# awslabs/flowgger

Hardware: AMD Instinct MI355X
Metric: log lines/sec (RFC5424, 256B avg) at 1/2/4/8 MI355X; achieved HBM GB/s (higher is better)
Workload: dtype u8

## Files before the change

flowgger_amd/csrc/fg_pipeline.hpp:

```cpp
#pragma once
#include "fg_device.hpp"
#include "fg_plan_policy.hpp"
#include "fg_sparse_need.hpp"
#include "fg_wave.hpp"

namespace fg {

using u32x4 = unsigned int __attribute__((ext_vector_type(4)));

__device__ __forceinline__ uint32_t eq_flags(uint32_t x, uint32_t pat) {
    uint32_t s = ((x & 0x7F7F7F7Fu) ^ pat) + 0x7F7F7F7Fu;
    return ~(s | x) & 0x80808080u;
}
__device__ __forceinline__ uint32_t range_flags(uint32_t x) {
    uint32_t l = x & 0x7F7F7F7Fu;
    uint32_t ge33 = l + 0x5F5F5F5Fu;
    uint32_t le126 = l + 0x01010101u;
    return ge33 & ~le126 & ~x & 0x80808080u;
}
__device__ __forceinline__ uint32_t ctrl_flags(uint32_t x) {
    uint32_t ge32 = (x & 0x7F7F7F7Fu) + 0x60606060u;
    return ~(ge32 | x) & 0x80808080u;
}
__device__ __forceinline__ uint32_t gather16(uint32_t f0, uint32_t f1, uint32_t f2, uint32_t f3) {
// ... 210 lines not shown
    uint32_t* ticket = nullptr;
    uint32_t ticket_base = 0;
    uint32_t taper0 = kNoTaper, taper1 = kNoTaper, taper2 = kNoTaper;
};

#define FG_STREAM_AUX 2
__device__ __forceinline__ uint4 stream_load(const uint4* p) {
    typedef uint32_t nt4 __attribute__((ext_vector_type(4)));
    const nt4 v = __builtin_nontemporal_load(reinterpret_cast<const nt4*>(p));
    return make_uint4(v.x, v.y, v.z, v.w);
}

template <class F, class = void>
struct tail_batch { static constexpr int value = 4; };
template <class F>
struct tail_batch<F, decltype((void)F::kTailBatch)> { static constexpr int value = F::kTailBatch; };

template <class F, class = void>
struct defer_row_store { static constexpr bool value = true; };
template <class F>
struct defer_row_store<F, decltype((void)F::kDeferRowStore)> { static constexpr bool value = F::kDeferRowStore; };

constexpr uint32_t kHeadCap = 1024;
template <class F, class = void>
struct head_cap { static constexpr uint32_t value = kHeadCap; };
template <class F>
struct head_cap<F, decltype((void)F::kHeadBytes)> { static constexpr uint32_t value = F::kHeadBytes; };

constexpr uint32_t kSparseHandful = 4;

template <int NB, bool PROF, class F, bool HEAD = false, uint32_t SPARSE = 0>
__device__ __forceinline__ void persistent_loop(const uint8_t* __restrict__ bytes, const uint64_t* __restrict__ offsets,
                                                uint64_t n, const DevTables& t, uint32_t tile_cap, uint32_t L, uint64_t chunk_lines,
                                                unsigned long long* prof, uint64_t* stash_base, F& fmt, FrameArgs fr) {
    static_assert(!HEAD || F::kClasses <= 1, "HEAD staging classifies one stage-A byte class at most");
    static_assert(SPARSE == 0 || (!HEAD && F::kClasses == 0), "the sparse window builds its need bitmap where a stage-A class bitmap would lie");
    static_assert(SPARSE % 16u == 0 && SPARSE <= 112u, "a line's run of chunks (at most (H + 4 + 14) / 16 + 1) must fit two bitmap words at any shift");
    const uint64_t kChunkLines = chunk_lines;
    extern __shared__ __attribute__((aligned(16))) uint8_t smem[];
    uint16_t* bm16 = reinterpret_cast<uint16_t*>(smem + tile_cap + 64u);
    const uint32_t bm_stride = tile_cap / 16u + 16u;
    uint4* dst = reinterpret_cast<uint4*>(smem);
    const uint32_t lane = threadIdx.x;
    const uint64_t G = gridDim.x;
    uint64_t* stash = stash_base ? stash_base + (uint64_t)blockIdx.x * (kStashEntries * kStashWords * kWave) : nullptr;

    const bool dyn = fr.ticket != nullptr;
    uint32_t tk_raw = 0;
    bool tk_pending = false;
    auto draw_ticket = [&]() {
        if (lane == 0u) tk_raw = __hip_atomic_fetch_add(fr.ticket, 1u, __ATOMIC_RELAXED, __HIP_MEMORY_SCOPE_AGENT);
        tk_pending = true;
    };
    uint64_t chunk = blockIdx.x;
    uint64_t p, hi_line;
    chunk_range(chunk, kChunkLines, fr.taper0, fr.taper1, fr.taper2, n, &p, &hi_line);
    if (dyn && p < n) draw_ticket();

    auto load_offsets = [&](uint64_t q, uint64_t* o0, uint64_t* o1) {
        const uint64_t li = q + lane;
        const bool in = lane < L && li < hi_line;
        *o0 = offsets[in ? li : hi_line];
        *o1 = offsets[in ? li + 1 : hi_line];
    };
    auto geometry = [&](uint64_t q, uint64_t o0, uint64_t o1, uint32_t* nl, uint64_t* a0, uint32_t* span) {
        const uint64_t left = hi_line - q;
        const uint32_t avail = left < (uint64_t)L ? (uint32_t)left : L;
        const uint32_t lo_l = (uint32_t)__builtin_amdgcn_readfirstlane((int)(uint32_t)o0);
        const uint32_t lo_h = (uint32_t)__builtin_amdgcn_readfirstlane((int)(uint32_t)(o0 >> 32));
        const uint64_t lo = (uint64_t)lo_l | ((uint64_t)lo_h << 32);
        *a0 = lo & ~15ull;
        const unsigned long long fit = __ballot(lane < avail && (o1 - *a0) <= (uint64_t)tile_cap);
        uint32_t cnt = fit == ~0ull ? 64u : (uint32_t)__builtin_ctzll(~fit);
        if (cnt == 0u) cnt = 1u;
        *nl = cnt;
        const uint32_t last = cnt - 1u;
        const uint32_t hi_l = (uint32_t)__builtin_amdgcn_readlane((int)(uint32_t)o1, (int)last);
        const uint32_t hi_h = (uint32_t)__builtin_amdgcn_readlane((int)(uint32_t)(o1 >> 32), (int)last);
        const uint64_t hi = (uint64_t)hi_l | ((uint64_t)hi_h << 32);
        const uint64_t want = hi - *a0;
        *span = want > tile_cap ? tile_cap : (uint32_t)((want + 15ull) & ~15ull);
    };
    auto load_window = [&](uint64_t a0, uint32_t span, u32x4* v) {
        __amdgpu_buffer_rsrc_t rsrc =
            __builtin_amdgcn_make_buffer_rsrc(const_cast<uint8_t*>(bytes + a0), (short)0, (int)span, 0x00020000);
#pragma unroll
        for (int k = 0; k < NB; ++k) v[k] = __builtin_amdgcn_raw_buffer_load_b128(rsrc, (int)(lane * 16u + k * 1024u), 0, FG_STREAM_AUX);
    };
    const uint32_t sparse_tail = fr.strip != FG_FRAME_NONE ? kSparseTailFramed : kSparseTailPlain;
// ... 70 lines not shown
    if (lane < 2u) ent_state[lane] = 0u;
    if (p >= hi_line) return;
    uint64_t o0, o1, a0 = 0;
    uint32_t span, nl, st = 0, tb = 0, last2 = 0;
    load_offsets(p, &o0, &o1);
    u32x4 v[NB];
    if constexpr (HEAD) {
        geometry_head(p, o0, o1, &nl, &span, &st, &tb);
        load_window_head(o0, st, v);
        last2 = load_last2(o0, o1);
    } else if constexpr (SPARSE != 0) {
        geometry(p, o0, o1, &nl, &a0, &span);
        uint32_t vo[NB];
        sparse_offsets(a0, span, nl, o0, o1, false, vo);
        load_window_sparse(a0, span, vo, v);
    } else {
        geometry(p, o0, o1, &nl, &a0, &span);
        load_window(a0, span, v);
    }
    bool dense = false, dense_next = false, dense_then = false;
    RowOut pend{};
    uint64_t pend_li = 0;
    bool pend_valid = false;
    uint64_t acc0 = 0, acc1 = 0, acc2 = 0, acc3 = 0, iters = 0, tm0 = 0, tm1 = 0, tm2 = 0, tm3 = 0;
    const uint32_t ablate = PROF ? (uint32_t)prof[5] : 0u;
    const uint32_t term4 = fr.strip == FG_FRAME_LINE ? 0x0A0A0A0Au : fr.strip == FG_FRAME_NUL ? 0u : wv::kNoTerm;

    for (;;) {
        uint64_t pn = p + nl;
        if (pn >= hi_line) {
            if (dyn) {
                if (!tk_pending) draw_ticket();
                const uint32_t tk = (uint32_t)__builtin_amdgcn_readfirstlane((int)tk_raw);
                chunk = (uint64_t)(uint32_t)(tk - fr.ticket_base) + G;
                tk_pending = false;
                chunk_range(chunk, kChunkLines, fr.taper0, fr.taper1, fr.taper2, n, &pn, &hi_line);
                if (pn < n) draw_ticket();
            } else {
                chunk += G;
                chunk_range(chunk, kChunkLines, kNoTaper, kNoTaper, kNoTaper, n, &pn, &hi_line);
            }
        }
        const bool more = pn < n;
        uint64_t no0 = 0, no1 = 0;
        if (more) load_offsets(pn, &no0, &no1);
        if (PROF) {
            tm0 = __builtin_amdgcn_s_memtime();
            __builtin_amdgcn_s_waitcnt(0x0F70);
            tm1 = __builtin_amdgcn_s_memtime();
        }
        FG_MARK(A);
        const uint32_t nchunk = span >> 4;
        const uint32_t nrow = HEAD ? nl : (nchunk + kWave - 1u) / kWave;
        if constexpr (HEAD) {
#pragma unroll
            for (int k = 0; k < NB; ++k) {
                if ((uint32_t)k < nl) {
                    const uint32_t tk = (uint32_t)__builtin_amdgcn_readlane((int)tb, k), sk = (uint32_t)__builtin_amdgcn_readlane((int)st, k);
                    if (lane * 16u < sk) {
                        const uint4 q = make_uint4(v[k][0], v[k][1], v[k][2], v[k][3]);
                        dst[(tk >> 4) + lane] = q;
                        if constexpr (F::kClasses != 0) F::classify_store(q, bm16, (tk >> 4) + lane, bm_stride, term4);
                    }
                }
            }
            constexpr uint32_t HB = tail_batch<F>::value >= 8 ? 8u : 4u;
            for (uint32_t r0 = NB; r0 < nl; r0 += HB) {
                uint4 w[HB];
                uint32_t tk[HB], sk[HB];
#pragma unroll
                for (uint32_t j = 0; j < HB; ++j) {
                    const uint32_t r = r0 + j < nl ? r0 + j : nl - 1u;
                    const uint32_t lo = (uint32_t)__builtin_amdgcn_readlane((int)(uint32_t)o0, (int)r);
                    const uint32_t hi = (uint32_t)__builtin_amdgcn_readlane((int)(uint32_t)(o0 >> 32), (int)r);
                    tk[j] = (uint32_t)__builtin_amdgcn_readlane((int)tb, (int)r);
                    sk[j] = (uint32_t)__builtin_amdgcn_readlane((int)st, (int)r);
                    const uint64_t b = ((uint64_t)lo | ((uint64_t)hi << 32)) & ~15ull;
                    __amdgpu_buffer_rsrc_t rsrc = __builtin_amdgcn_make_buffer_rsrc(const_cast<uint8_t*>(bytes + b), (short)0, (int)sk[j], 0x00020000);
                    const u32x4 x = __builtin_amdgcn_raw_buffer_load_b128(rsrc, (int)(lane * 16u), 0, FG_STREAM_AUX);
                    w[j] = make_uint4(x[0], x[1], x[2], x[3]);
                }
#pragma unroll
                for (uint32_t j = 0; j < HB; ++j)
                    if (lane * 16u < sk[j]) {
                        dst[(tk[j] >> 4) + lane] = w[j];
                        if constexpr (F::kClasses != 0) F::classify_store(w[j], bm16, (tk[j] >> 4) + lane, bm_stride, term4);
                    }
            }
        } else {
#pragma unroll
        for (int k = 0; k < NB; ++k) {
            if ((uint32_t)k < nrow) {
                uint32_t idx = k * kWave + lane;
                uint4 q = make_uint4(v[k][0], v[k][1], v[k][2], v[k][3]);
                dst[idx] = q;
                F::classify_store(q, bm16, idx, bm_stride, idx < nchunk ? term4 : wv::kPastSpan);
            }
        }
        }
        if (!HEAD && nrow > (uint32_t)NB) {
            const uint4* __restrict__ src = reinterpret_cast<const uint4*>(bytes + a0);
            const uint32_t last = nchunk - 1u;
            constexpr int TB = tail_batch<F>::value;
            for (uint32_t c0 = NB * kWave; c0 < nchunk; c0 += kWave * TB) {
                uint4 w[TB];
#pragma unroll
                for (int k = 0; k < TB; ++k) {
                    const uint32_t idx = c0 + k * kWave + lane;
                    w[k] = stream_load(src + (idx < last ? idx : last));
                }
#pragma unroll
                for (int k = 0; k < TB; ++k) {
                    if (k == 0 || c0 + k * kWave < nchunk) {
                        const uint32_t idx = c0 + k * kWave + lane, ci = idx < last ? idx : last;
                        dst[ci] = w[k];
                        F::classify_store(w[k], bm16, ci, bm_stride, term4);
                    }
                }
            }
            if constexpr (SPARSE != 0) __builtin_amdgcn_s_waitcnt(0x0F70);
        }
        __builtin_amdgcn_sched_barrier(0);
        FG_MARK(S);
        if (PROF) {
            __builtin_amdgcn_s_waitcnt(0xC07F);
// ... 261 lines not shown
```

flowgger_amd/csrc/fg_plan_policy.hpp:

```cpp
#pragma once
#include <stdint.h>

#include "../../include/fg_hip.h"
#include "fg_sparse_need.hpp"

#if defined(__HIPCC__)
#define FG_POLICY_HD __host__ __device__
#else
#define FG_POLICY_HD
#endif

namespace fg {

constexpr uint32_t kNoTaper = 0xFFFFFFFFu;

FG_POLICY_HD inline void chunk_range(uint64_t c, uint64_t chunk, uint32_t t0, uint32_t t1, uint32_t t2, uint64_t n, uint64_t* lo,
                                     uint64_t* hi) {
    uint64_t base = 0, first = 0, sz = chunk;
    if (c >= t0) {
        base = (uint64_t)t0 * sz, first = t0, sz >>= 1;
        if (c >= t1) {
            base += (uint64_t)(t1 - t0) * sz, first = t1, sz >>= 1;
            if (c >= t2) base += (uint64_t)(t2 - t1) * sz, first = t2, sz >>= 1;
        }
// ... 54 lines not shown
        if (chunk < L) chunk = L;
    }
    if (chunk < 1u) chunk = 1u;
    p.chunk = chunk;
    p.chunks = (n + chunk - 1) / chunk;
    if (lo.flags & (FG_LO_TAPER_1 | FG_LO_TAPER_2)) taper = ((lo.flags & FG_LO_TAPER_1) ? 1u : 0u) + ((lo.flags & FG_LO_TAPER_2) ? 2u : 0u);
    if (taper > 3u) taper = 3u;
    if (tickets && taper && !(lo.flags & FG_LO_NO_TAPER)) {
        uint64_t m = n / (2u * chunk);
        if (m > blocks) m = blocks;
        uint32_t levels = 0;
        while (levels < taper && (chunk >> (levels + 1u)) >= g) ++levels;
        if (m >= 1u && levels >= 1u && p.chunks + 4u * m < 0xFFFFFFF0ull) {
            const uint64_t t0 = (n - m * chunk) / chunk;
            p.taper[0] = (uint32_t)t0;
            if (levels >= 2u) p.taper[1] = (uint32_t)(t0 + m);
            if (levels >= 3u) p.taper[2] = (uint32_t)(t0 + 2u * m);
            p.chunks = count_chunks(chunk, p.taper, n);
        }
    }
    p.blocks = (uint32_t)(blocks > p.chunks ? p.chunks : blocks);
    p.tickets = tickets;
    return p;
}

constexpr int kWindowKiB = 20;
constexpr uint32_t kMaxTile = 57344;

constexpr uint32_t tile_lds(uint32_t tile, uint32_t classes = 1) { return tile + 64u + (tile / 16u + 16u) * 2u * classes; }

constexpr uint32_t kShortLineTile = 17408;
static_assert(tile_lds(kShortLineTile) <= 160u * 1024u / 8u, "eight waves per CU");
static_assert(tile_lds(kShortLineTile + 1024u) > 160u * 1024u / 8u, "the largest such tile");

constexpr uint64_t kHeadFromLen = 768, kPairsFromLen = 320;
struct Variant { bool head, pairs; };
inline Variant pick_variant(uint64_t avg_len, uint32_t flags) {
    return Variant{(flags & FG_LO_FORCE_HEAD) || (avg_len >= kHeadFromLen && !(flags & FG_LO_NO_HEAD)),
                   (flags & FG_LO_SD_PAIRS) || (avg_len >= kPairsFromLen && !(flags & FG_LO_SD_WALK))};
}
#if !defined(FG_SPARSE_DEFAULT)
#define FG_SPARSE_DEFAULT 1
#endif
constexpr bool kSparseDefault = FG_SPARSE_DEFAULT != 0;
inline bool pick_sparse(uint64_t avg_len, uint32_t flags, const Variant& v) {
    if (v.head || v.pairs) return false;
    return (flags & FG_LO_FORCE_SPARSE) || (kSparseDefault && avg_len >= kSparseFromLen && !(flags & FG_LO_NO_SPARSE));
}
inline bool gelf_group_fits_3k(uint64_t avg_len) { return 8u * avg_len * 17u / 16u + 256u <= 3072u; }
inline bool gelf_const_3k(uint64_t avg_len, const fg_launch_opts& lo) {
    return gelf_group_fits_3k(avg_len) && !lo.tile_cap && !(lo.flags & FG_LO_GELF_GENERIC);
}

struct PlanFormat {
    uint32_t max_lines = 64;
    uint32_t n_classes = 1;
    uint32_t (*extra_for)(uint32_t tile, uint32_t lines) = nullptr;
    uint32_t (*extra_tile)(uint32_t tile) = nullptr;
    uint32_t default_tile = 0;
    uint32_t default_chunk = 0;
    uint32_t ticket_from = 2;
    uint32_t taper = 1;
    PlanFormat& lines(uint32_t v) { max_lines = v; return *this; }
    PlanFormat& classes(uint32_t v) { n_classes = v; return *this; }
    PlanFormat& lds_for(uint32_t (*f)(uint32_t, uint32_t)) { extra_for = f; return *this; }
    PlanFormat& lds_tile(uint32_t (*f)(uint32_t)) { extra_tile = f; return *this; }
// ... 73 lines not shown
```

flowgger_amd/csrc/fg_rfc5424.hip:

```cpp
#include <cstdio>
#include <cstdlib>

#include "fg_fused.hpp"
#include "fg_sd2.hpp"
#include "fg_tsfast.hpp"

namespace fg {

enum : uint32_t {
    E_OK = 0,
    E_BOM = 1,
    E_BRACKETS = 2,
    E_INVPRI = 3,
    E_NOVER = 4,
    E_BADVER = 5,
    E_NOTS = 6,
    E_BADTS = 7,
    E_NOHOST = 8,
    E_NOAPP = 9,
    E_NOPROC = 10,
    E_NOMSGID = 11,
    E_NODATA = 12,
    E_NOMSG = 13,
    E_MALFORMED = 14,
    E_NOSD = 15,
    E_SDFMT = 16,
    E_NOBRACKET = 17
};

struct Row {
    uint32_t status = E_OK;
    uint32_t facility = 0xFF, severity = 0xFF, flags = 0;
    double ts = 0.0;
    uint32_t off[6];
    uint32_t len[6];
    uint32_t data0 = 0;
    uint32_t n_ent = 0;
};


template <class R>
__device__ __forceinline__ uint32_t find_space(R& rd, uint32_t q, uint32_t len) {
    while (q < len && rd.byte(q) != ' ') ++q;
    return q;
}

template <bool EMIT, class R>
__device__ __forceinline__ uint32_t sd_walk(R& rd, uint32_t pos, uint32_t len, uint32_t* msg_at, uint32_t* n_ent,
                            const DevTables& t, uint32_t slot) {
    uint32_t cnt = 0;
    for (;;) {
        uint32_t s = pos + 1;
        uint32_t sp = find_space(rd, s, len);
        if (sp >= len) return E_NOSD;
        if (EMIT) {
            t.ent_name[slot + cnt] = fg_span{s, sp - s};
            t.ent_val[slot + cnt] = 0;
            t.ent_type[slot + cnt] = FG_T_SDID;
            t.ent_flags[slot + cnt] = 0;
        }
        ++cnt;
        uint32_t st = 0, name_s = 0, name_e = 0, val_s = 0, esc_seen = 0;
        uint32_t i = sp + 1;
        uint32_t after = 0;
        for (; i < len; ++i) {
            uint32_t c = rd.byte(i);
            if (st == 3) {
                if (c == '\\') {
                    st = 4;
                    esc_seen = 1;
                } else if (c == '"') {
                    if (EMIT) {
                        t.ent_name[slot + cnt] = fg_span{name_s, name_e - name_s};
                        t.ent_val[slot + cnt] = (uint64_t)val_s | ((uint64_t)(i - val_s) << 32);
                        t.ent_type[slot + cnt] = FG_T_STRING;
                        t.ent_flags[slot + cnt] = esc_seen ? FG_EF_VAL_ESC : 0;
                    }
                    ++cnt;
                    st = 0;
                }
            } else if (st == 4) {
                st = 3;
            } else {
                bool is_name = (c - 33u) <= 93u && c != '"' && c != '=' && c != ']';
                if (st == 0) {
                    if (c == ' ' || c == '"') {
                    } else if (c == ']') {
                        after = i + 1;
                        break;
                    } else if (is_name) {
                        st = 1;
                        name_s = i;
                    } else {
                        return E_SDFMT;
                    }
                } else if (st == 1) {
                    if (is_name) {
                    } else if (c == '=') {
                        name_e = i;
                        st = 2;
                    } else {
                        return E_SDFMT;
                    }
                } else {
                    if (c != '"') return E_SDFMT;
                    st = 3;
                    val_s = i + 1;
                    esc_seen = 0;
                }
// ... 142 lines not shown
struct Fast {
    uint32_t route;
    uint32_t no_ts;
    uint32_t ts_ok;
    uint32_t rest;
    uint32_t t0, te;
    uint32_t d0;
    uint32_t c7;
    uint32_t e, s;
    uint32_t start_ok;
};

__device__ __forceinline__ uint32_t fast_rfc3339(const Tile& T, uint32_t base, const uint32_t* hdr, uint32_t t0, uint32_t L,
                                                 double* out) {
    const uint32_t a = base + t0;
    const uint32_t s = t0 - 4u;
    uint32_t r[9];
#pragma unroll
    for (int k = 0; k < 9; ++k) r[k] = __builtin_amdgcn_alignbyte(hdr[k + 2], hdr[k + 1], s);
    return fast_rfc3339_core(r, L, [&](uint32_t pos, uint32_t* z0, uint32_t* z1) { load8(T, a + pos, z0, z1); }, out);
}

__device__ __forceinline__ uint32_t take_space(uint64_t& lo, uint64_t& hi, uint32_t none, uint32_t& found) {
    const bool in_lo = lo != 0, in_hi = hi != 0;
    const uint32_t p = in_lo ? (uint32_t)__builtin_ctzll(lo) : in_hi ? 64u + (uint32_t)__builtin_ctzll(hi) : none;
    const uint64_t lo2 = lo & (lo - 1ull), hi2 = hi & (hi - 1ull);
    hi = in_lo ? hi : hi2;
    lo = lo2;
    found += (in_lo || in_hi) ? 1u : 0u;
    return p;
}

constexpr uint32_t kNoLastByte = 0xFFFFFFFFu;
__device__ __forceinline__ Fast parse_line_fast(const Tile& T, uint32_t base, uint32_t len, Row& r, uint32_t last_byte, uint32_t vis) {
    Fast f;
    uint32_t l0 = last_byte, l1;
    if (last_byte == kNoLastByte) load8(T, base + (len ? len - 1u : 0u), &l0, &l1);
    uint32_t hdr[33];
    {
        const uint32_t d = base >> 2, sft = base & 3u;
        uint32_t raw[34];
#pragma unroll
        for (int k = 0; k < 34; ++k) raw[k] = T.w[d + k];
#pragma unroll
        for (int k = 0; k < 33; ++k) hdr[k] = __builtin_amdgcn_alignbyte(raw[k + 1], raw[k], sft);
    }
    const uint32_t h0 = hdr[0], h1 = hdr[1];

    const uint32_t c1 = ((h0 >> 8) & 0xFFu) - '0', c2 = ((h0 >> 16) & 0xFFu) - '0', c3 = (h0 >> 24) - '0';
    const bool d2 = c2 <= 9u, d3 = d2 && c3 <= 9u;
    const uint32_t nd = 1u + (d2 ? 1u : 0u) + (d3 ? 1u : 0u);
    uint32_t pri = c1;
    pri = d2 ? pri * 10u + c2 : pri;
    pri = d3 ? pri * 10u + c3 : pri;
    const uint64_t hh = (((uint64_t)h1 << 32) | h0) >> (8u * (1u + nd));
    const uint32_t sp0 = 3u + nd;
    const bool shape = (h0 & 0xFFu) == '<' && c1 <= 9u && pri <= 255u && (uint32_t)(hh & 0xFFFFu) == (('1' << 8) | '>') &&
                       sp0 <= len;
    f.no_ts = sp0 == len ? 1u : 0u;
    f.route = (!shape || (sp0 < len && (uint32_t)((hh >> 16) & 0xFFu) != ' ')) ? R_GENERIC : 0u;
    r.facility = pri >> 3;
    r.severity = pri & 7u;

    uint64_t lo, hi;
    {
        uint32_t m[8];
#pragma unroll
        for (int k = 0; k < 8; ++k)
            m[k] = gather16(eq_flags(hdr[4 * k], 0x20202020u), eq_flags(hdr[4 * k + 1], 0x20202020u),
                            eq_flags(hdr[4 * k + 2], 0x20202020u), eq_flags(hdr[4 * k + 3], 0x20202020u));
        lo = (uint64_t)(m[0] | (m[1] << 16)) | ((uint64_t)(m[2] | (m[3] << 16)) << 32);
        hi = (uint64_t)(m[4] | (m[5] << 16)) | ((uint64_t)(m[6] | (m[7] << 16)) << 32);
    }
    {
        const uint64_t lo_keep = vis < 64u ? (1ull << (vis & 63u)) - 1ull : ~0ull;
        const uint64_t hi_keep = vis < 64u ? 0ull : vis < 128u ? (1ull << ((vis - 64u) & 63u)) - 1ull : ~0ull;
        lo &= lo_keep & ~((2ull << sp0) - 1ull);
        hi &= hi_keep;
    }
    uint32_t found = 0;
    const uint32_t s1 = take_space(lo, hi, len, found);
    const uint32_t s2 = take_space(lo, hi, len, found);
    const uint32_t s3 = take_space(lo, hi, len, found);
    const uint32_t s4 = take_space(lo, hi, len, found);
    const uint32_t s5 = take_space(lo, hi, len, found);
    f.route |= (found < 5u && len > 128u) ? R_GENERIC : 0u;

    f.t0 = sp0 + 1u;
    f.te = s1;
    {
        const uint32_t ok = fast_rfc3339(T, base, hdr, f.t0, s1 - f.t0, &r.ts);
        f.ts_ok = ok == 1u ? 1u : 0u;
        f.route |= ok == 2u ? R_TS_SLOW : 0u;
    }
    r.off[S_HOST] = s1 + 1u;
    r.len[S_HOST] = s2 - s1 - 1u;
    r.off[S_APP] = s2 + 1u;
    r.len[S_APP] = s3 - s2 - 1u;
    r.off[S_PROC] = s3 + 1u;
    r.len[S_PROC] = s4 - s3 - 1u;
    r.off[S_MSGID] = s4 + 1u;
    r.len[S_MSGID] = s5 - s4 - 1u;
    const uint32_t d0 = s5 + 1u;
    f.d0 = d0;
    f.rest = found < 5u ? E_NOHOST + found : d0 >= len ? E_NOMSG : E_OK;

    uint32_t m0, m1;
    load8(T, base + (d0 < len ? d0 : 0u), &m0, &m1);
    const uint32_t c = m0 & 0xFFu;
    f.c7 = c;
    const bool live = !f.no_ts && f.rest == E_OK;
    f.route |= (live && c != '-') ? R_TAIL : 0u;
    const uint32_t last = l0 & 0xFFu;
    const bool end_plain = last > 0x20u && last < 0x80u;
    f.e = len;
    const uint32_t cA = (m0 >> 8) & 0xFFu, cB = (m0 >> 16) & 0xFFu;
    const uint32_t s = d0 + 1u;
    const bool one_sp = s + 1u < len && cA == ' ' && cB > 0x20u && cB < 0x80u;
    const bool no_sp = s < len && cA > 0x20u && cA < 0x80u;
// ... 50 lines not shown
    constexpr bool EMIT = MODE == SD_EMIT;
    LdsReader rd(T.w, base);
    uint32_t cnt = 0;
    uint32_t wpos = (base + 3u) & ~3u;
    bool rec_ok = true;
    auto record = [&](uint64_t rec, uint32_t consumed) {
        if (rec_ok) {
            if (wpos + 8u <= base + consumed) {
                tile_w[wpos >> 2] = (uint32_t)rec;
                tile_w[(wpos >> 2) + 1u] = (uint32_t)(rec >> 32);
                wpos += 8u;
            } else {
                rec_ok = false;
            }
        }
    };
    for (;;) {
        const uint32_t s = pos + 1;
        uint32_t sp = s;
        for (;;) {
            if (sp >= len) return E_NOSD;
            uint32_t w[4];
            load16(T, base + sp, w);
            const uint32_t avail = len - sp < 16u ? len - sp : 16u;
            const uint32_t hit = gather16(eq_flags(w[0], 0x20202020u), eq_flags(w[1], 0x20202020u), eq_flags(w[2], 0x20202020u),
                                          eq_flags(w[3], 0x20202020u)) & ((1u << avail) - 1u);
            if (hit) {
                sp += (uint32_t)__builtin_ctz(hit);
                break;
            }
            sp += avail;
        }
        if (EMIT) {
            t.ent_name[slot + cnt] = fg_span{s, sp - s};
            t.ent_val[slot + cnt] = 0;
            t.ent_type[slot + cnt] = FG_T_SDID;
            t.ent_flags[slot + cnt] = 0;
        }
        if (MODE == SD_STASH) record(stash_pack(s, sp - s, 0, 0, 1), sp + 1u);
        ++cnt;
        uint32_t status = E_OK;
        uint32_t i = sp + 1;
        bool in_value = false;
        uint32_t name_s = 0, name_e = 0, val_s = 0, cur = 0, esc_seen = 0;
        uint32_t close_at = 0;
        for (;;) {
            uint32_t w0 = i, start = 0;
            if (in_value) {
                const uint32_t p = find_bit(T.bm, base, cur, len);
                if (p >= len) {
                    status = E_NOBRACKET;
                    break;
                }
                w0 = p;
                start = 1;
            } else if (i >= len) {
                status = E_NOBRACKET;
                break;
            }
            uint32_t w[4];
            load16(T, base + w0, w);
            if (in_value) {
                if ((w[0] & 0xFFu) == '\\') {
                    esc_seen = 1;
                    cur = w0 + 2;
                    continue;
                }
                if (EMIT) {
                    t.ent_name[slot + cnt] = fg_span{name_s, name_e - name_s};
                    t.ent_val[slot + cnt] = (uint64_t)val_s | ((uint64_t)(w0 - val_s) << 32);
                    t.ent_type[slot + cnt] = FG_T_STRING;
                    t.ent_flags[slot + cnt] = esc_seen ? FG_EF_VAL_ESC : 0;
                }
                if (MODE == SD_STASH) record(stash_pack(name_s, name_e - name_s, w0 - val_s, esc_seen, 0), w0 + 1u);
                ++cnt;
                in_value = false;
            }
            const uint32_t avail = len - w0 < 16u ? len - w0 : 16u;
            const uint32_t inside = (1u << avail) - 1u;
            const WinMasks m = window_masks(w);
            const uint32_t from = ~((1u << start) - 1u);
            const uint32_t stop = ~m.skip & from & inside;
            if (stop == 0) {
                i = w0 + avail;
                continue;
            }
            const uint32_t i0 = (uint32_t)__builtin_ctz(stop);
            if ((m.rb >> i0) & 1u) {
                close_at = w0 + i0;
                break;
            }
            if (!((m.name >> i0) & 1u)) {
                status = E_SDFMT;
                break;
            }
            const uint32_t after_name = ~m.name & ~((1u << i0) - 1u) & 0xFFFFu;
            const uint32_t e0 = after_name ? (uint32_t)__builtin_ctz(after_name) : 16u;
            if (e0 + 1u < avail) {
                if (!((m.eq >> e0) & 1u) || !((m.quote >> (e0 + 1u)) & 1u)) {
                    status = E_SDFMT;
                    break;
                }
                name_s = w0 + i0;
                name_e = w0 + e0;
                val_s = name_e + 2u;
// ... 105 lines not shown
    const bool valid = c.valid;
    uint64_t* stash = c.stash;
    const uint32_t lane = threadIdx.x;
    Row r;
#pragma unroll
    for (int k = 0; k < 6; ++k) {
        r.off[k] = 0;
        r.len[k] = FG_NONE;
    }
    const uint32_t len = (uint32_t)(o1 - o0);
    const bool in_window = !kSparse || (o1 - a0) <= (uint64_t)span;
    const bool in_tile = HEAD ? c.tlen == len && in_window : (o1 - a0) <= (uint64_t)span;
    const bool head_only = HEAD && !in_tile && (kSparse ? in_window : c.tlen >= 512u);
    const uint32_t walk_len = HEAD ? c.tlen : len;
    const uint32_t sd_len = kSparse ? len : walk_len;
    const uint32_t base = HEAD ? c.tbase : (uint32_t)(o0 - a0);
    bool from_global = false;
    uint32_t* tile_w = reinterpret_cast<uint32_t*>(const_cast<uint8_t*>(smem));
    bool rec_ok = false;
    Tile T{reinterpret_cast<const uint32_t*>(smem), reinterpret_cast<const uint32_t*>(bm16)};
    uint64_t pc[10] = {0, 0, 0, 0, 0, 0, 0, 0, 0, 0}, tk = PROF ? wv::clock() : 0;
    auto tick = [&](int k) {
        if (PROF) {
            const uint64_t now = wv::clock();
            pc[k] += now - tk;
            tk = now;
        }
    };
    uint32_t route = 0;
    Fast f{};
    if (valid) {
        route = R_GENERIC;
        if (in_tile || head_only) {
            f = parse_line_fast(T, base, len, r, HEAD ? (len ? (c.last2 & 0xFFu) : 0u) : kNoLastByte, kSparse ? walk_len : len);
            route = f.route;
            if (kSparse && head_only && f.d0 + 3u > walk_len) route |= R_GENERIC;
            if (!(route & R_GENERIC)) {
                if (route & R_TS_SLOW) {
                    LdsReader rd(T.w, base);
                    bool ok = parse_rfc3339(rd, f.t0, f.te, &r.ts);
                    r.status = f.no_ts ? E_NOTS : ok ? f.rest : E_BADTS;
                } else {
                    r.status = f.no_ts ? E_NOTS : f.ts_ok ? f.rest : E_BADTS;
                }
            }
        }
    }
    const bool sd_any = valid && !(route & R_GENERIC) && (route & R_TAIL) && r.status == E_OK && f.c7 == '[' && !(kSparse && head_only);
    const uint64_t sd_ballot = __ballot(sd_any);
    const bool group_has_sd = __any(sd_any && len - f.d0 > kShortSdTail) || __popcll(sd_ballot) > 4;
    const bool sd_lane = sd_any && group_has_sd;
    if constexpr (!NESTED) FG_MARK(F);
    tick(0);
    sd2::Lds SL{};
    sd2::LineIn sin{false, 0u, 0u, 0u, false};
    sd2::LineOut slo{false, 0u, false, E_OK, 0u, 0u, 0u};
    bool sd2_ran = false;
    if constexpr (SDX) {
        if (group_has_sd) {
            const uint32_t stride16 = c.tile_cap / 16u + 16u;
            SL = sd2::carve(smem, bm16, c.tile_cap, reinterpret_cast<uint8_t*>(bm16 + 2u * stride16));
            __syncthreads();
            const bool chain = sd2::classify_tile(SL, span);
            __syncthreads();
            tick(1);
            sin = sd2::LineIn{sd_lane && (in_tile || head_only), base, f.d0, walk_len, in_tile};
            if (!chain) {
// ... 104 lines not shown
    tick(6);
    uint32_t first = 0;
    {
        const EntAlloc ea = alloc_entries_ex(t, r.n_ent, c.ent_state);
        tick(7);
        const uint32_t mine = (ea.overflow || ea.total == 0u) ? 0u : ea.s.at(ea.ex);
        if (ea.overflow) {
            r.status = FG_ST_OVERFLOW;
            r.n_ent = 0;
        }
        first = r.n_ent != 0 ? mine : 0u;
        const bool by_pairs = SDX && sd_lane && slo.handled && !from_global;
        if constexpr (SDX) {
            if (sd2_ran) sd2::group_emit(SL, t, sin, slo, by_pairs && !ea.overflow && !(ablate & 4u), first);
        }
        if (r.n_ent != 0 && !(ablate & 4u) && !by_pairs) {
            uint32_t msg_at, cnt;
            if (sd_lane && !from_global && stash && rec_ok) {
                const uint32_t* rec32 = tile_w + (((base + 3u) & ~3u) >> 2);
                for (uint32_t k0 = 0; k0 < r.n_ent; k0 += 4u) {
                    uint32_t lo[4], hi[4];
#pragma unroll
                    for (uint32_t j = 0; j < 4u; ++j) {
                        const uint32_t k = k0 + j < r.n_ent ? k0 + j : r.n_ent - 1u;
                        lo[j] = rec32[k * 2u];
                        hi[j] = rec32[k * 2u + 1u];
                    }
#pragma unroll
                    for (uint32_t j = 0; j < 4u; ++j) {
                        const uint32_t k = k0 + j;
                        if (k < r.n_ent) {
                            const uint32_t name_s = lo[j] & 0xFFFFu, name_len = lo[j] >> 16, val_len = hi[j] & 0xFFFFu;
                            const bool sdid = (hi[j] >> 17) & 1u;
                            t.ent_name[first + k] = fg_span{name_s, name_len};
                            t.ent_val[first + k] = sdid ? 0ull : ((uint64_t)(name_s + name_len + 2u) | ((uint64_t)val_len << 32));
                            t.ent_type[first + k] = sdid ? FG_T_SDID : FG_T_STRING;
                            t.ent_flags[first + k] = ((hi[j] >> 16) & 1u) ? FG_EF_VAL_ESC : 0;
                        }
                    }
                }
            } else if (from_global || (sd_lane && stash)) {
                FG_RARE_BEGIN();
                GlobalReader rd(reinterpret_cast<const uint32_t*>(bytes), o0);
                sd_walk<true>(rd, r.data0, len, &msg_at, &cnt, t, first);
                FG_RARE_END();
            } else if (sd_lane) {
                sd_walk_tile<SD_EMIT>(T, base, r.data0, sd_len, &msg_at, &cnt, t, first);
            } else if (in_tile) {
                LdsReader rd(T.w, base);
                sd_walk<true>(rd, r.data0, len, &msg_at, &cnt, t, first);
            } else {
                FG_RARE_BEGIN();
                GlobalReader rd(reinterpret_cast<const uint32_t*>(bytes), o0);
                sd_walk<true>(rd, r.data0, len, &msg_at, &cnt, t, first);
                FG_RARE_END();
            }
        }
    }

    tick(8);
    RowOut o;
    const bool ok = r.status == E_OK;
    o.meta = r.status | (r.facility << 8) | (r.severity << 16) | (r.flags << 24);
    o.ts = ok ? r.ts : 0.0;
#pragma unroll
    for (int k = 0; k < 6; ++k) o.span[k] = ok ? fg_span{r.off[k], r.len[k]} : fg_span{0, FG_NONE};
    o.first = first;
    o.count = r.n_ent;
    if constexpr (kSparse) {
        o.handed = valid && in_window && (coop ||
// ... 53 lines not shown
    tick(9);
    if (PROF && pacc && lane == 0)
        for (int k = 0; k < 10; ++k) pacc[k] += (unsigned long long)pc[k];
    return o;
    }
};

using Rfc5424Format = Rfc5424FormatT<false>;

template <int NB, bool PROF, bool HEAD = false, bool SDX = false>
__global__ __launch_bounds__(kWave, 2) void k_rfc5424(const uint8_t* __restrict__ bytes,
                                                     const uint64_t* __restrict__ offsets, uint64_t n, DevTables t,
                                                     uint32_t tile_cap, uint32_t L, uint64_t groups,
                                                     unsigned long long* prof, uint64_t* stash_base, FrameArgs fr) {
    Rfc5424FormatT<HEAD, SDX, PROF> fmt;
    if constexpr (PROF) {
        __shared__ unsigned long long pacc[10];
        if (threadIdx.x < 10) pacc[threadIdx.x] = 0ull;
        fmt.pacc = pacc;
        __syncthreads();
        persistent_loop<NB, PROF, Rfc5424FormatT<HEAD, SDX, PROF>, HEAD>(bytes, offsets, n, t, tile_cap, L, groups, prof, stash_base, fmt, fr);
        __syncthreads();
        if (prof && threadIdx.x < 10) atomicAdd(&prof[6 + threadIdx.x], pacc[threadIdx.x]);
    } else if constexpr (SDX) {
        __shared__ DevTables t_lds;
        if (threadIdx.x == 0) t_lds = t;
        __syncthreads();
        persistent_loop<NB, PROF, Rfc5424FormatT<HEAD, SDX, PROF>, HEAD>(bytes, offsets, n, t_lds, tile_cap, L, groups, prof, stash_base, fmt, fr);
    } else {
        persistent_loop<NB, PROF, Rfc5424FormatT<HEAD, SDX, PROF>, HEAD>(bytes, offsets, n, t, tile_cap, L, groups, prof, stash_base, fmt, fr);
    }
}

template <int NB, bool PROF, uint32_t H>
__global__ __launch_bounds__(kWave, 2) void k_rfc5424_sparse(const uint8_t* __restrict__ bytes, const uint64_t* __restrict__ offsets, uint64_t n,
                                                            DevTables t, uint32_t tile_cap, uint32_t L, uint64_t groups,
                                                            unsigned long long* prof, uint64_t* stash_base, FrameArgs fr) {
    Rfc5424FormatT<true, false, PROF, H> fmt;
    if constexpr (PROF) {
        __shared__ unsigned long long pacc[10];
        if (threadIdx.x < 10) pacc[threadIdx.x] = 0ull;
        fmt.pacc = pacc;
        __syncthreads();
        persistent_loop<NB, PROF, Rfc5424FormatT<true, false, PROF, H>, false, H>(bytes, offsets, n, t, tile_cap, L, groups, prof, stash_base, fmt, fr);
        __syncthreads();
        if (prof && threadIdx.x < 10) atomicAdd(&prof[6 + threadIdx.x], pacc[threadIdx.x]);
    } else {
        persistent_loop<NB, PROF, Rfc5424FormatT<true, false, PROF, H>, false, H>(bytes, offsets, n, t, tile_cap, L, groups, prof, stash_base, fmt, fr);
    }
}

template <int NB, bool SDX>
__global__ __launch_bounds__(kWave, 2) void k_rfc5424_fused(const uint8_t* __restrict__ bytes, DevTables t, uint32_t tile_cap, uint32_t L,
                                                           uint64_t* stash_base, FusedArgs fa, uint32_t strip) {
    Rfc5424FormatT<false, SDX, false> fmt;
    __shared__ DevTables t_lds;
    __shared__ FusedArgs fa_lds;
    if (threadIdx.x == 0) {
        t_lds = t;
        fa_lds = fa;
    }
    __syncthreads();
    fused_loop<NB>(bytes, t_lds, tile_cap, L, fmt, fa_lds, strip, stash_base);
}

}

extern "C" uint64_t fg_stash_bytes(uint32_t blocks) {
    return (uint64_t)blocks * fg::kStashEntries * fg::kStashWords * fg::kWave * sizeof(uint64_t);
}

namespace {
template <bool HEAD, bool SDX>
auto rfc5424_kernels(const char* name) {
    return fg::kernels(fg::k_rfc5424<fg::kWindowKiB, false, HEAD, SDX>, FG_PROF_TWIN(fg::k_rfc5424<fg::kWindowKiB, true, HEAD, SDX>), name);
}
}

extern "C" int fg_launch_rfc5424(const uint8_t* d_bytes, const uint64_t* d_offsets, uint64_t n, const fg::DevTables* t,
                                 uint64_t avg_len, hipStream_t stream, uint64_t* stash, uint32_t stash_blocks, uint32_t strip,
                                 const uint8_t* line_bad, const fg_launch_opts* lo, fg::TicketSlot* tk) {
// ... 34 lines not shown
```

Baseline: 18.35 billion.

## Stage sparse kernel args in LDS and shrink fast header parse window

```diff
diff --git a/flowgger_amd/csrc/fg_pipeline.hpp b/flowgger_amd/csrc/fg_pipeline.hpp
--- a/flowgger_amd/csrc/fg_pipeline.hpp
+++ b/flowgger_amd/csrc/fg_pipeline.hpp
@@ -266,7 +266,7 @@
 template <int NB, bool PROF, class F, bool HEAD = false, uint32_t SPARSE = 0>
 __device__ __forceinline__ void persistent_loop(const uint8_t* __restrict__ bytes, const uint64_t* __restrict__ offsets,
                                                 uint64_t n, const DevTables& t, uint32_t tile_cap, uint32_t L, uint64_t chunk_lines,
-                                                unsigned long long* prof, uint64_t* stash_base, F& fmt, FrameArgs fr) {
+                                                unsigned long long* prof, uint64_t* stash_base, F& fmt, FrameArgs fr, const FrameArgs* fr_lds = nullptr) {
     static_assert(!HEAD || F::kClasses <= 1, "HEAD staging classifies one stage-A byte class at most");
     static_assert(SPARSE == 0 || (!HEAD && F::kClasses == 0), "the sparse window builds its need bitmap where a stage-A class bitmap would lie");
     static_assert(SPARSE % 16u == 0 && SPARSE <= 112u, "a line's run of chunks (at most (H + 4 + 14) / 16 + 1) must fit two bitmap words at any shift");
@@ -280,15 +280,20 @@
     uint64_t* stash = stash_base ? stash_base + (uint64_t)blockIdx.x * (kStashEntries * kStashWords * kWave) : nullptr;
 
     const bool dyn = fr.ticket != nullptr;
+    const FrameArgs& fc = SPARSE != 0 ? *fr_lds : fr;
     uint32_t tk_raw = 0;
     bool tk_pending = false;
     auto draw_ticket = [&]() {
-        if (lane == 0u) tk_raw = __hip_atomic_fetch_add(fr.ticket, 1u, __ATOMIC_RELAXED, __HIP_MEMORY_SCOPE_AGENT);
+        if constexpr (SPARSE != 0) {
+            if (lane == 0u) tk_raw = __hip_atomic_fetch_add((uint32_t __attribute__((address_space(1)))*)fc.ticket, 1u, __ATOMIC_RELAXED, __HIP_MEMORY_SCOPE_AGENT);
+        } else {
+            if (lane == 0u) tk_raw = __hip_atomic_fetch_add(fr.ticket, 1u, __ATOMIC_RELAXED, __HIP_MEMORY_SCOPE_AGENT);
+        }
         tk_pending = true;
     };
     uint64_t chunk = blockIdx.x;
     uint64_t p, hi_line;
-    chunk_range(chunk, kChunkLines, fr.taper0, fr.taper1, fr.taper2, n, &p, &hi_line);
+    chunk_range(chunk, kChunkLines, fc.taper0, fc.taper1, fc.taper2, n, &p, &hi_line);
     if (dyn && p < n) draw_ticket();
 
     auto load_offsets = [&](uint64_t q, uint64_t* o0, uint64_t* o1) {
@@ -425,9 +430,9 @@
             if (dyn) {
                 if (!tk_pending) draw_ticket();
                 const uint32_t tk = (uint32_t)__builtin_amdgcn_readfirstlane((int)tk_raw);
-                chunk = (uint64_t)(uint32_t)(tk - fr.ticket_base) + G;
+                chunk = (uint64_t)(uint32_t)(tk - fc.ticket_base) + G;
                 tk_pending = false;
-                chunk_range(chunk, kChunkLines, fr.taper0, fr.taper1, fr.taper2, n, &pn, &hi_line);
+                chunk_range(chunk, kChunkLines, fc.taper0, fc.taper1, fc.taper2, n, &pn, &hi_line);
                 if (pn < n) draw_ticket();
             } else {
                 chunk += G;
@@ -481,9 +486,12 @@
                     }
             }
         } else {
+        uint32_t nrow_a = nrow;
+        if constexpr (SPARSE != 0) asm("s_mov_b32 %0, %1" : "=s"(nrow_a) : "s"(nrow));
 #pragma unroll
         for (int k = 0; k < NB; ++k) {
-            if ((uint32_t)k < nrow) {
+            const bool in = (uint32_t)k < nrow_a;
+            if (SPARSE != 0 ? (bool)__builtin_expect(in, true) : in) {
                 uint32_t idx = k * kWave + lane;
                 uint4 q = make_uint4(v[k][0], v[k][1], v[k][2], v[k][3]);
                 dst[idx] = q;
diff --git a/flowgger_amd/csrc/fg_plan_policy.hpp b/flowgger_amd/csrc/fg_plan_policy.hpp
--- a/flowgger_amd/csrc/fg_plan_policy.hpp
+++ b/flowgger_amd/csrc/fg_plan_policy.hpp
@@ -110,6 +110,8 @@
 constexpr uint32_t kShortLineTile = 17408;
 static_assert(tile_lds(kShortLineTile) <= 160u * 1024u / 8u, "eight waves per CU");
 static_assert(tile_lds(kShortLineTile + 1024u) > 160u * 1024u / 8u, "the largest such tile");
+constexpr uint32_t kSparseStaticLds = 256;
+static_assert(tile_lds(kShortLineTile) + kSparseStaticLds <= 160u * 1024u / 8u, "eight waves per CU, the sparse kernel's static LDS included");
 
 constexpr uint64_t kHeadFromLen = 768, kPairsFromLen = 320;
 struct Variant { bool head, pairs; };
diff --git a/flowgger_amd/csrc/fg_rfc5424.hip b/flowgger_amd/csrc/fg_rfc5424.hip
--- a/flowgger_amd/csrc/fg_rfc5424.hip
+++ b/flowgger_amd/csrc/fg_rfc5424.hip
@@ -54,10 +54,10 @@
         uint32_t sp = find_space(rd, s, len);
         if (sp >= len) return E_NOSD;
         if (EMIT) {
-            t.ent_name[slot + cnt] = fg_span{s, sp - s};
-            t.ent_val[slot + cnt] = 0;
-            t.ent_type[slot + cnt] = FG_T_SDID;
-            t.ent_flags[slot + cnt] = 0;
+            gstore(t.ent_name, slot + cnt, fg_span{s, sp - s});
+            gstore(t.ent_val, slot + cnt, (uint64_t)(0));
+            gstore(t.ent_type, slot + cnt, (uint8_t)(FG_T_SDID));
+            gstore(t.ent_flags, slot + cnt, (uint8_t)(0));
         }
         ++cnt;
         uint32_t st = 0, name_s = 0, name_e = 0, val_s = 0, esc_seen = 0;
@@ -71,10 +71,10 @@
                     esc_seen = 1;
                 } else if (c == '"') {
                     if (EMIT) {
-                        t.ent_name[slot + cnt] = fg_span{name_s, name_e - name_s};
-                        t.ent_val[slot + cnt] = (uint64_t)val_s | ((uint64_t)(i - val_s) << 32);
-                        t.ent_type[slot + cnt] = FG_T_STRING;
-                        t.ent_flags[slot + cnt] = esc_seen ? FG_EF_VAL_ESC : 0;
+                        gstore(t.ent_name, slot + cnt, fg_span{name_s, name_e - name_s});
+                        gstore(t.ent_val, slot + cnt, (uint64_t)((uint64_t)val_s | ((uint64_t)(i - val_s) << 32)));
+                        gstore(t.ent_type, slot + cnt, (uint8_t)(FG_T_STRING));
+                        gstore(t.ent_flags, slot + cnt, (uint8_t)(esc_seen ? FG_EF_VAL_ESC : 0));
                     }
                     ++cnt;
                     st = 0;
@@ -283,18 +283,21 @@
 }
 
 constexpr uint32_t kNoLastByte = 0xFFFFFFFFu;
+template <uint32_t W = 128>
 __device__ __forceinline__ Fast parse_line_fast(const Tile& T, uint32_t base, uint32_t len, Row& r, uint32_t last_byte, uint32_t vis) {
+    static_assert(W % 16u == 0 && W >= 80u && W <= 128u, "whole 16-byte classes; the timestamp's registers (hdr[1..10]) and the two mask words");
+    constexpr int NW = (int)(W / 4u);
     Fast f;
     uint32_t l0 = last_byte, l1;
     if (last_byte == kNoLastByte) load8(T, base + (len ? len - 1u : 0u), &l0, &l1);
-    uint32_t hdr[33];
+    uint32_t hdr[NW + 1];
     {
         const uint32_t d = base >> 2, sft = base & 3u;
-        uint32_t raw[34];
-#pragma unroll
-        for (int k = 0; k < 34; ++k) raw[k] = T.w[d + k];
-#pragma unroll
-        for (int k = 0; k < 33; ++k) hdr[k] = __builtin_amdgcn_alignbyte(raw[k + 1], raw[k], sft);
+        uint32_t raw[NW + 2];
+#pragma unroll
+        for (int k = 0; k < NW + 2; ++k) raw[k] = T.w[d + k];
+#pragma unroll
+        for (int k = 0; k < NW + 1; ++k) hdr[k] = __builtin_amdgcn_alignbyte(raw[k + 1], raw[k], sft);
     }
     const uint32_t h0 = hdr[0], h1 = hdr[1];
 
@@ -315,9 +318,9 @@
 
     uint64_t lo, hi;
     {
-        uint32_t m[8];
-#pragma unroll
-        for (int k = 0; k < 8; ++k)
+        uint32_t m[8] = {0, 0, 0, 0, 0, 0, 0, 0};
+#pragma unroll
+        for (int k = 0; k < NW / 4; ++k)
             m[k] = gather16(eq_flags(hdr[4 * k], 0x20202020u), eq_flags(hdr[4 * k + 1], 0x20202020u),
                             eq_flags(hdr[4 * k + 2], 0x20202020u), eq_flags(hdr[4 * k + 3], 0x20202020u));
         lo = (uint64_t)(m[0] | (m[1] << 16)) | ((uint64_t)(m[2] | (m[3] << 16)) << 32);
@@ -335,7 +338,7 @@
     const uint32_t s3 = take_space(lo, hi, len, found);
     const uint32_t s4 = take_space(lo, hi, len, found);
     const uint32_t s5 = take_space(lo, hi, len, found);
-    f.route |= (found < 5u && len > 128u) ? R_GENERIC : 0u;
+    f.route |= (found < 5u && len > W) ? R_GENERIC : 0u;
 
     f.t0 = sp0 + 1u;
     f.te = s1;
@@ -452,10 +455,10 @@
             sp += avail;
         }
         if (EMIT) {
-            t.ent_name[slot + cnt] = fg_span{s, sp - s};
-            t.ent_val[slot + cnt] = 0;
-            t.ent_type[slot + cnt] = FG_T_SDID;
-            t.ent_flags[slot + cnt] = 0;
+            gstore(t.ent_name, slot + cnt, fg_span{s, sp - s});
+            gstore(t.ent_val, slot + cnt, (uint64_t)(0));
+            gstore(t.ent_type, slot + cnt, (uint8_t)(FG_T_SDID));
+            gstore(t.ent_flags, slot + cnt, (uint8_t)(0));
         }
         if (MODE == SD_STASH) record(stash_pack(s, sp - s, 0, 0, 1), sp + 1u);
         ++cnt;
@@ -487,10 +490,10 @@
                     continue;
                 }
                 if (EMIT) {
-                    t.ent_name[slot + cnt] = fg_span{name_s, name_e - name_s};
-                    t.ent_val[slot + cnt] = (uint64_t)val_s | ((uint64_t)(w0 - val_s) << 32);
-                    t.ent_type[slot + cnt] = FG_T_STRING;
-                    t.ent_flags[slot + cnt] = esc_seen ? FG_EF_VAL_ESC : 0;
+                    gstore(t.ent_name, slot + cnt, fg_span{name_s, name_e - name_s});
+                    gstore(t.ent_val, slot + cnt, (uint64_t)((uint64_t)val_s | ((uint64_t)(w0 - val_s) << 32)));
+                    gstore(t.ent_type, slot + cnt, (uint8_t)(FG_T_STRING));
+                    gstore(t.ent_flags, slot + cnt, (uint8_t)(esc_seen ? FG_EF_VAL_ESC : 0));
                 }
                 if (MODE == SD_STASH) record(stash_pack(name_s, name_e - name_s, w0 - val_s, esc_seen, 0), w0 + 1u);
                 ++cnt;
@@ -662,7 +665,7 @@
     if (valid) {
         route = R_GENERIC;
         if (in_tile || head_only) {
-            f = parse_line_fast(T, base, len, r, HEAD ? (len ? (c.last2 & 0xFFu) : 0u) : kNoLastByte, kSparse ? walk_len : len);
+            f = parse_line_fast<kSparse ? HB : 128u>(T, base, len, r, HEAD ? (len ? (c.last2 & 0xFFu) : 0u) : kNoLastByte, kSparse ? walk_len : len);
             route = f.route;
             if (kSparse && head_only && f.d0 + 3u > walk_len) route |= R_GENERIC;
             if (!(route & R_GENERIC)) {
@@ -833,10 +836,10 @@
                         if (k < r.n_ent) {
                             const uint32_t name_s = lo[j] & 0xFFFFu, name_len = lo[j] >> 16, val_len = hi[j] & 0xFFFFu;
                             const bool sdid = (hi[j] >> 17) & 1u;
-                            t.ent_name[first + k] = fg_span{name_s, name_len};
-                            t.ent_val[first + k] = sdid ? 0ull : ((uint64_t)(name_s + name_len + 2u) | ((uint64_t)val_len << 32));
-                            t.ent_type[first + k] = sdid ? FG_T_SDID : FG_T_STRING;
-                            t.ent_flags[first + k] = ((hi[j] >> 16) & 1u) ? FG_EF_VAL_ESC : 0;
+                            gstore(t.ent_name, first + k, fg_span{name_s, name_len});
+                            gstore(t.ent_val, first + k, (uint64_t)(sdid ? 0ull : ((uint64_t)(name_s + name_len + 2u) | ((uint64_t)val_len << 32))));
+                            gstore(t.ent_type, first + k, (uint8_t)(sdid ? FG_T_SDID : FG_T_STRING));
+                            gstore(t.ent_flags, first + k, (uint8_t)(((hi[j] >> 16) & 1u) ? FG_EF_VAL_ESC : 0));
                         }
                     }
                 }
@@ -956,21 +959,33 @@
     }
 }
 
+struct SparseStatics {
+    DevTables t;
+    FrameArgs fr;
+};
 template <int NB, bool PROF, uint32_t H>
 __global__ __launch_bounds__(kWave, 2) void k_rfc5424_sparse(const uint8_t* __restrict__ bytes, const uint64_t* __restrict__ offsets, uint64_t n,
                                                             DevTables t, uint32_t tile_cap, uint32_t L, uint64_t groups,
                                                             unsigned long long* prof, uint64_t* stash_base, FrameArgs fr) {
     Rfc5424FormatT<true, false, PROF, H> fmt;
+    __shared__ __attribute__((aligned(16))) uint8_t st_raw[sizeof(SparseStatics)];
+    SparseStatics& st_lds = *reinterpret_cast<SparseStatics*>(st_raw);
+    static_assert(sizeof(SparseStatics) <= kSparseStaticLds, "the static LDS of the sparse kernel beside the largest short-line tile");
+    if (threadIdx.x == 0) {
+        st_lds.t = t;
+        st_lds.fr = fr;
+    }
+    __syncthreads();
     if constexpr (PROF) {
         __shared__ unsigned long long pacc[10];
         if (threadIdx.x < 10) pacc[threadIdx.x] = 0ull;
         fmt.pacc = pacc;
         __syncthreads();
-        persistent_loop<NB, PROF, Rfc5424FormatT<true, false, PROF, H>, false, H>(bytes, offsets, n, t, tile_cap, L, groups, prof, stash_base, fmt, fr);
+        persistent_loop<NB, PROF, Rfc5424FormatT<true, false, PROF, H>, false, H>(bytes, offsets, n, st_lds.t, tile_cap, L, groups, prof, stash_base, fmt, fr, &st_lds.fr);
         __syncthreads();
         if (prof && threadIdx.x < 10) atomicAdd(&prof[6 + threadIdx.x], pacc[threadIdx.x]);
     } else {
-        persistent_loop<NB, PROF, Rfc5424FormatT<true, false, PROF, H>, false, H>(bytes, offsets, n, t, tile_cap, L, groups, prof, stash_base, fmt, fr);
+        persistent_loop<NB, PROF, Rfc5424FormatT<true, false, PROF, H>, false, H>(bytes, offsets, n, st_lds.t, tile_cap, L, groups, prof, stash_base, fmt, fr, &st_lds.fr);
     }
 }
 
```

After: 18.32 billion. About the same (-0.2%).
